# miguelmartin75/txt2vid

Measured on AMD Instinct MI355X. Metric: TGANv2 GAN train throughput (G+D steps x global batch), 16x64x64 videos/sec, higher is better.
Workload: dtype f32; 1 GPU; BASELINE configs[1]: unconditional TGANv2 16x64x64x1, per-GPU batch 32, fp32, RSGAN + GP 0.5, Adam 2e-4 (0.5,0.999), 1 D + 1 G step, subsample_input pyramid 8/16/32/64; global_batch=32, per_gpu_batch=32, parallelism=dp1

## Files before the change

include/t2v_hip.h:

```cpp
#ifndef T2V_HIP_H
#define T2V_HIP_H

#include <stddef.h>
#include <stdint.h>

#ifdef __cplusplus
extern "C" {
#endif

#define T2V_OK 0
#define T2V_EINVAL (-1)
#define T2V_ELAUNCH (-2)

#define T2V_MAX_TAPS 27

typedef struct {
    int32_t N, Cin, D, H, W, Cout;
    int32_t ntaps;
    int8_t dz[T2V_MAX_TAPS], dy[T2V_MAX_TAPS], dx[T2V_MAX_TAPS];
    int8_t pad_[3];
} t2v_conv_geom;

#define T2V_MAX_GROUPS 8
typedef struct {
// ... 53 lines not shown
typedef struct {
    const float* slab;
    const float* bias_slab;
    int32_t ntaps, S;
    int8_t map[T2V_MAX_TAPS];
    int8_t pad_[5];
    int64_t tap_stride;
    int64_t split_stride;
} t2v_wgrad_src;
typedef struct {
    float* dw;
    float* dbias;
    int64_t CoCi;
    int32_t T, Cout, nsrc;
    int32_t accum, accum_bias;
    int32_t kind;
    int32_t block_begin, nblocks;
    int32_t tap_major;
    int32_t pad_;
    t2v_wgrad_src src[T2V_WGRAD_MAX_SRC];
} t2v_wgrad_dest;
int t2v_conv_wgrad_grouped_partial(const t2v_conv_group* groups, int ngroups, int Cin, int Cout, int kD, int kH, int kW,
                                   float* slab, int want_bias, int flags, t2v_wgrad_src* out_src, void* stream);
int t2v_wgrad_dest_bytes(void);
int t2v_wgrad_reduce_multi(const void* table , int ndest, int total_blocks, void* stream);

int t2v_conv_fwd_plan(const t2v_conv_group* groups, int ngroups, int Cin, int Cout, int flags, int32_t* out);
int t2v_conv_wgrad_plan(const t2v_conv_group* groups, int ngroups, int Cin, int Cout, int kD, int kH, int kW, int32_t* out);
int64_t t2v_conv_wgrad_grouped_bias_slab_floats(const t2v_conv_group* groups, int ngroups, int Cin, int Cout, int kD,
                                                int kH, int kW);
int t2v_conv_wgrad_grouped_bias(const t2v_conv_group* groups, int ngroups, int Cin, int Cout, int kD, int kH, int kW,
                                float* dw, float* dbias, float* slab, int flags, void* stream);

int t2v_pack_weight_bf16(const float* w, void* wpb, int Cout, int Cin, int T, const int32_t* taps, int ntaps, int mode, void* stream);
int t2v_conv_fwd_grouped_bf16_ok(const t2v_conv_group* groups, int ngroups, int Cin, int Cout);
int t2v_conv_fwd_bf16_plan(const t2v_conv_group* groups, int ngroups, int Cin, int Cout, int flags, int32_t* out);
int t2v_conv_fwd_grouped_bf16(const t2v_conv_group* groups, int ngroups, int Cin, int Cout, const void* wpb, const float* bias,
                              float* ws, int flags, void* stream);

int64_t t2v_channel_sum_ws_floats(int N, int C, int64_t S);
int t2v_channel_sum(const float* x, float* out, float* ws, int N, int C, int64_t S, int accum, void* stream);
int64_t t2v_channel_sum_grouped_ws_floats(const t2v_conv_group* groups, int ngroups, int C);
int t2v_channel_sum_grouped(const t2v_conv_group* groups, int ngroups, int C, float* out, float* ws, int accum, void* stream);

int t2v_relu(const float* x, float* y, int64_t n, void* stream);
int t2v_relu_mask(const float* g, const float* x, float* gx, int64_t n, void* stream);
int t2v_add(const float* a, const float* b, float* y, int64_t n, void* stream);
int t2v_axpby(float alpha, const float* a, float beta, const float* b, float* y, int64_t n, void* stream);
int t2v_fill(float* y, float v, int64_t n, void* stream);
int t2v_tanh(const float* x, float* y, int64_t n, void* stream);
int t2v_tanh_bwd(const float* g, const float* y, float* gx, int64_t n, void* stream);

int t2v_avgpool3d(const float* x, const float* x2, float* y, int NC, int D, int H, int W, int Do, int Ho, int Wo,
                  const int32_t k[3], const int32_t s[3], const int32_t p[3], void* stream);
int t2v_avgpool3d_bwd(const float* gy, float* gx, int NC, int D, int H, int W, int Do, int Ho, int Wo,
                      const int32_t k[3], const int32_t s[3], const int32_t p[3], void* stream);
typedef struct t2v_pool_job {
    const float* x; const float* x2; float* y;
    const float* add;
    int32_t NC, D, H, W, Do, Ho, Wo;
    int32_t k[3], s[3], p[3];
} t2v_pool_job;
int t2v_avgpool3d_multi(const t2v_pool_job* jobs, int njobs, void* stream);
int t2v_avgpool3d_bwd_multi(const t2v_pool_job* jobs, int njobs, void* stream);

int t2v_rowsum(const float* x, float* y, int64_t rows, int64_t S, void* stream);
// ... 293 lines not shown
```

txt2vid_amd/_lib.py:

```python
import ctypes as C
import os

_HERE = os.path.dirname(os.path.abspath(__file__))
LIB_PATH = os.environ.get('T2V_LIB') or os.path.join(_HERE, 'csrc', 'libt2v_hip.so')

MAX_TAPS = 27


class ConvGeom(C.Structure):
    _fields_ = [('N', C.c_int32), ('Cin', C.c_int32), ('D', C.c_int32), ('H', C.c_int32), ('W', C.c_int32),
                ('Cout', C.c_int32), ('ntaps', C.c_int32),
                ('dz', C.c_int8 * MAX_TAPS), ('dy', C.c_int8 * MAX_TAPS), ('dx', C.c_int8 * MAX_TAPS),
                ('pad_', C.c_int8 * 3)]


class ConvGroup(C.Structure):
    _fields_ = [('x', C.c_void_p), ('y', C.c_void_p), ('mask', C.c_void_p), ('N', C.c_int32), ('D', C.c_int32), ('H', C.c_int32), ('W', C.c_int32),
                ('ntaps', C.c_int32), ('dstride', C.c_int32), ('ydstride', C.c_int32), ('yoff', C.c_int32), ('Dy', C.c_int32),
                ('dz', C.c_int8 * MAX_TAPS), ('dy', C.c_int8 * MAX_TAPS), ('dx', C.c_int8 * MAX_TAPS), ('widx', C.c_int8 * MAX_TAPS)]


class AdamJob(C.Structure):
    _fields_ = [('p', C.c_void_p), ('g', C.c_void_p), ('m', C.c_void_p), ('v', C.c_void_p), ('n', C.c_int64)]

# ... 78 lines not shown
_L = C.c_int64
_F = C.c_float
_I3 = C.POINTER(C.c_int32)
_G = C.POINTER(ConvGeom)

SIGNATURES = {
    't2v_pack_weight': [_P, _P, _I, _I, _I, _I3, _I, _I, _P],
    't2v_pack_job_bytes': [],
    't2v_pack_multi': [_P, _I, _I, _P],
    't2v_pack_job_groups': [_I, _I, _I],
    't2v_pack_weight_into': [_P, _P, _I, _I, _I, _I3, _I, _I, _I, _I, _I, _I, _P],
    't2v_conv_fwd': [_P, _P, _P, _P, _P, _G, _I, _P],
    't2v_conv_fwd_ws_floats': [_G],
    't2v_conv_wgrad_slab_floats': [_G, _I],
    't2v_conv_fwd_grouped_ws_floats': [_P, _I, _I, _I],
    't2v_conv_fwd_grouped': [_P, _I, _I, _I, _P, _P, _P, _I, _P],
    't2v_conv_wgrad_grouped_slab_floats': [_P, _I, _I, _I, _I, _I, _I],
    't2v_conv_fwd_plan': [_P, _I, _I, _I, _I, _I3],
    't2v_nonlocal_ok': [_I, _I],
    't2v_nonlocal_fwd': [_P, _P, _P, _P, _P, _I, _I, _I, _I, _I, _P],
    't2v_nonlocal_bwd': [_P, _P, _P, _P, _P, _P, _P, _P, _P, _P, _I, _I, _I, _I, _I, _P],
    't2v_conv_wgrad_grouped_partial': [_P, _I, _I, _I, _I, _I, _I, _P, _I, _I, _P, _P],
    't2v_wgrad_dest_bytes': [],
    't2v_wgrad_reduce_multi': [_P, _I, _I, _P],
    't2v_conv_wgrad_plan': [_P, _I, _I, _I, _I, _I, _I, _I3],
    't2v_pack_weight_bf16': [_P, _P, _I, _I, _I, _P, _I, _I, _P],
    't2v_conv_fwd_grouped_bf16_ok': [_P, _I, _I, _I],
    't2v_conv_fwd_bf16_plan': [_P, _I, _I, _I, _I, _I3],
    't2v_conv_fwd_grouped_bf16': [_P, _I, _I, _I, _P, _P, _P, _I, _P],
    't2v_conv_wgrad_grouped': [_P, _I, _I, _I, _I, _I, _I, _P, _P, _I, _P],
    't2v_conv_wgrad_grouped_bias_slab_floats': [_P, _I, _I, _I, _I, _I, _I],
    't2v_conv_wgrad_grouped_bias': [_P, _I, _I, _I, _I, _I, _I, _P, _P, _P, _I, _P],
    't2v_conv_wgrad': [_P, _P, _P, _P, _G, _I3, _I, _I, _P],
    't2v_channel_sum_ws_floats': [_I, _I, _L],
    't2v_channel_sum': [_P, _P, _P, _I, _I, _L, _I, _P],
    't2v_channel_sum_grouped_ws_floats': [_P, _I, _I],
    't2v_channel_sum_grouped': [_P, _I, _I, _P, _P, _I, _P],
    't2v_relu': [_P, _P, _L, _P],
    't2v_relu_mask': [_P, _P, _P, _L, _P],
    't2v_add': [_P, _P, _P, _L, _P],
    't2v_axpby': [_F, _P, _F, _P, _P, _L, _P],
    't2v_fill': [_P, _F, _L, _P],
    't2v_tanh': [_P, _P, _L, _P],
    't2v_tanh_bwd': [_P, _P, _P, _L, _P],
    't2v_avgpool3d': [_P, _P, _P, _I, _I, _I, _I, _I, _I, _I, _I3, _I3, _I3, _P],
    't2v_avgpool3d_bwd': [_P, _P, _I, _I, _I, _I, _I, _I, _I, _I3, _I3, _I3, _P],
    't2v_avgpool3d_multi': [_P, _I, _P],
    't2v_avgpool3d_bwd_multi': [_P, _I, _P],
    't2v_rowsum': [_P, _P, _L, _L, _P],
    't2v_rowbcast': [_P, _P, _L, _L, _P],
    't2v_upsample2x': [_P, _P, _L, _I, _I, _P],
    't2v_upsample2x_bwd': [_P, _P, _L, _I, _I, _P],
    't2v_upsample2x_add': [_P, _P, _P, _L, _I, _I, _P],
    't2v_rsgan_mean_multi': [_P, _I, _P, _P],
    't2v_rsgan_mean_multi_bwd': [_P, _I, _P, _P],
    't2v_bn_ws_floats': [_I, _I, _L],
    't2v_bn_plan': [_I, _I, _L, _I3],
    't2v_bn_stats': [_P, _P, _P, _P, _P, _I, _I, _L, _F, _F, _P],
    't2v_bn_apply': [_P, _P, _P, _P, _P, _I, _I, _L, _I, _P],
    't2v_bn_bwd': [_P, _P, _P, _P, _P, _P, _P, _P, _P, _I, _I, _L, _I, _P],
    't2v_bn_train_fwd': [_P, _P, _P, _P, _P, _P, _P, _P, _I, _I, _L, _F, _F, _I, _P, _P],
    't2v_bn_train_bwd': [_P, _P, _P, _P, _P, _P, _P, _P, _P, _I, _I, _L, _I, _P],
    't2v_bn_train_fwd_up': [_P, _P, _P, _P, _P, _P, _P, _P, _I, _I, _I, _I, _F, _F, _I, _P, _P],
    't2v_bn_train_bwd_up': [_P, _P, _P, _P, _P, _P, _P, _P, _P, _I, _I, _I, _I, _I, _P],
    't2v_bn_train_bwd_add': [_P, _P, _P, _P, _P, _P, _P, _P, _P, _P, _I, _I, _I, _I, _I, _I, _P],
    't2v_bn_eval': [_P, _P, _P, _P, _P, _P, _I, _I, _L, _F, _I, _P],
# ... 74 lines not shown
    't2v_pool_conv_plan': [_I, _P, _I, _I, _I, _I3],
    't2v_synth_clips': [_P, _I, _L, _I, _I, _I, _I3, _P, _P, _P, _P],
    't2v_clip_gather': [_P, _L, _P, _I, _I, _I, _I, _I, _P, _P, _P, _P],
    't2v_tseed_fwd_bn': [_P, _P, _P, _P, _P, _P, _P, _P, _P, _P, _P, _I, _I, _I, _I, _I, _F, _F, _I, _P],
    't2v_tseed_fwd_tanh': [_P, _P, _P, _P, _P, _I, _I, _I, _I, _P],
    't2v_tseed_bwd': [_P, _P, _P, _P, _P, _P, _P, _P, _P, _P, _I, _I, _I, _I, _I, _I, _P],
    't2v_ca_fwd': [_P, _P, _P, _P, _P, _I, _I, _I, _P],
    't2v_ca_bwd': [_P, _P, _F, _P, _P, _P, _I, _I, _I, _P],
    't2v_diffaug_fwd': [_P, _I, _P],
    't2v_diffaug_bwd': [_P, _I, _P],
    't2v_diffaug_gated_fwd': [_P, _P, _I, _P, _P],
    't2v_diffaug_gated_bwd': [_P, _P, _I, _P, _P],
    't2v_ada_update': [_P, _P, _I, _F, _F, _I, _P],
    't2v_lecam_fwd': [_P, _P, _I, _F, _I, _P, _P, _P],
    't2v_lecam_bwd': [_P, _I, _P, _P, _P],
    't2v_proj_rows': [_P, _I, _P, _I, _I, _P],
    't2v_proj_feat': [_P, _I, _P, _I, _I, _P],
    't2v_proj_cond': [_P, _I, _P, _I, _I, _P],
    't2v_proj_weight': [_P, _I, _P, _I, _I, _I, _P],
    't2v_mbstd_fwd': [_P, _I, _P, _I, _I, _I, _P],
    't2v_mbstd_feat': [_P, _I, _P, _I, _I, _I, _P],
    't2v_mbstd_second': [_P, _I, _P, _I, _I, _I, _P],
    't2v_mbstd_weight': [_P, _I, _P, _I, _I, _I, _I, _P],
    't2v_kid_sums': [_P, _P, _I, _I, _I, C.c_double, _P, _P, _P],
    't2v_kid_sums_ws_bytes': [_I, _I, _I],
    't2v_knn_radii': [_P, _I, _I, _I, _P, _P, _P],
    't2v_knn_radii_ws_bytes': [_I, _I, _I],
    't2v_prdc_counts': [_P, _P, _I, _I, _I, _P, _P, _P, _P, _P],
    't2v_prdc_counts_ws_bytes': [_I, _I, _I],
    't2v_prof_begin': [_I],
    't2v_prof_end': [C.POINTER(C.c_double), _I],
    't2v_version': [],
}
_RESTYPE = {'t2v_kid_sums_ws_bytes': C.c_size_t, 't2v_knn_radii_ws_bytes': C.c_size_t, 't2v_prdc_counts_ws_bytes': C.c_size_t, 't2v_multi_ws_floats': C.c_int64, 't2v_sn_ws_floats': C.c_int64, 't2v_pool_conv_fwd_ws_floats': C.c_int64, 't2v_pool_conv_wgrad_slab_floats': C.c_int64, 't2v_conv_wgrad_slab_floats': C.c_int64, 't2v_conv_wgrad_grouped_bias_slab_floats': C.c_int64, 't2v_conv_fwd_grouped_ws_floats': C.c_int64,
            't2v_conv_wgrad_grouped_slab_floats': C.c_int64, 't2v_conv_fwd_ws_floats': C.c_int64, 't2v_channel_sum_ws_floats': C.c_int64, 't2v_channel_sum_grouped_ws_floats': C.c_int64, 't2v_bn_ws_floats': C.c_int64, 't2v_cbn_ws_floats': C.c_int64, 't2v_version': C.c_char_p}

_lib = None


class T2VError(RuntimeError):
    pass


def lib():
    global _lib
    if _lib is None:
        if not os.path.exists(LIB_PATH):
            raise T2VError('libt2v_hip.so is missing (%s): run `python -c "import __graft_entry__ as g; g.build()"` '
                           'or `make -C txt2vid_amd/csrc`. There is no CPU/PyTorch fallback.' % LIB_PATH)
        import torch
        l = C.CDLL(LIB_PATH)
        for name, argtypes in SIGNATURES.items():
            fn = getattr(l, name)
            fn.argtypes = argtypes
            fn.restype = _RESTYPE.get(name, C.c_int)
        _lib = l
    return _lib


def check(status, what):
    if status != 0:
        raise T2VError('%s failed with status %d' % (what, status))
```

txt2vid_amd/csrc/conv.hip:

```cpp
#include <hip/hip_runtime.h>
#include <stdint.h>
#include "../../include/t2v_hip.h"

typedef float f32x16 __attribute__((ext_vector_type(16)));

#ifdef T2V_STAMPS
__device__ unsigned long long* g_stamps = nullptr;
__device__ unsigned int g_stamps_cap = 0;
extern "C" int t2v_stamps_set(void* buf, unsigned int cap_records) {
    if (hipMemcpyToSymbol(HIP_SYMBOL(g_stamps), &buf, sizeof(buf)) != hipSuccess) return -1;
    if (hipMemcpyToSymbol(HIP_SYMBOL(g_stamps_cap), &cap_records, sizeof(cap_records)) != hipSuccess) return -1;
    return 0;
}
__device__ __forceinline__ unsigned long long stamp_now() {
    unsigned long long t;
    __builtin_amdgcn_sched_barrier(0);
    asm volatile("s_memtime %0\n\ts_waitcnt lgkmcnt(0)" : "=s"(t) :: "memory");
    __builtin_amdgcn_sched_barrier(0);
    return t;
}
#define STAMP(v) const unsigned long long v = stamp_now()
#define STAMP_ACC(acc, a, b) acc += (b) - (a)
#else
#define STAMP(v)
// ... 3532 lines not shown
                acc = __builtin_amdgcn_mfma_f32_32x32x2f32(a4[i].w, b4[i].w, acc, 0, 0, 0);
            }
        }
        __syncthreads();
    }
    float* red = As;
    if (wk == 1) {
#pragma unroll
        for (int r = 0; r < 16; ++r) red[(wco * 16 + r) * 64 + lane] = acc[r];
    }
    __syncthreads();
    if (wk == 0) {
#pragma unroll
        for (int r = 0; r < 16; ++r) acc[r] += red[(wco * 16 + r) * 64 + lane];
        const int col = l31;
        if (col < ncols) {
            const int slot = col / Cin, ci = col - slot * Cin;
            float* ps = slab + ((size_t)split * live.n + slot) * Cout * Cin + ci;
#pragma unroll
            for (int r = 0; r < 16; ++r) {
                const int co = co0 + wco * 32 + (r & 3) + 8 * (r >> 2) + 4 * hi;
                if (co < Cout) ps[(size_t)co * Cin] = acc[r];
            }
        } else if (col == 31 && bias_slab != nullptr) {
#pragma unroll
            for (int r = 0; r < 16; ++r) {
                const int co = co0 + wco * 32 + (r & 3) + 8 * (r >> 2) + 4 * hi;
                if (co < Cout) bias_slab[(size_t)split * Cout + co] = acc[r];
            }
        }
    }
}

#define W3_AP (WG_BK + 1)
#define W3_BP (WG_BK + 3)
struct LiveRows { int8_t r[9]; int32_t n; };

#define W3_XP (WG_BK + 3)

template <bool BF16>
__global__ __launch_bounds__(256, BF16 ? 4 : 0) void conv_wgrad3_kernel(const WGroupTable tab, float* __restrict__ slab, const int Cin,
                                                          const int Cout, const int kD, const int kH, const int flags,
                                                          const int chunks_per_split, const LiveRows live,
                                                          float* __restrict__ bias_slab) {
    constexpr int LDS_A = BF16 ? 64 * B16_KP * 2 : 64 * W3_AP * 4;
    constexpr int LDS_B = BF16 ? 3 * 64 * B16_KP * 2 : 3 * 64 * W3_XP * 4;
    __shared__ __attribute__((aligned(16))) unsigned char lds_raw[LDS_A + LDS_B];
    float* const As = reinterpret_cast<float*>(lds_raw);
    float* const Bs = reinterpret_cast<float*>(lds_raw + LDS_A);
    __bf16* const Ah = reinterpret_cast<__bf16*>(lds_raw);
    __bf16* const Bh = reinterpret_cast<__bf16*>(lds_raw + LDS_A);
    const int tid = threadIdx.x, lane = tid & 63, wave = tid >> 6;
    const int l31 = lane & 31, hi = lane >> 5;
    const int wco = wave & 1, wci = wave >> 1;
    const int nco_t = (Cout + 63) / 64;
    const int co0 = (blockIdx.x % nco_t) * 64, ci0 = (blockIdx.x / nco_t) * 64;
    const int lin = xcd_remap((int)(blockIdx.y + blockIdx.z * gridDim.y), (int)(gridDim.y * gridDim.z));
    const int rslot = lin % (int)gridDim.y;
    const int split = lin / (int)gridDim.y;
    const int krow = live.r[rslot];
    const int dz = krow / kH - kD / 2, dy = krow % kH - kH / 2;
    const float relu_floor = (flags & T2V_CONV_RELU_IN) ? 0.f : -__builtin_inff();
    const int ml = tid & 31, rl = tid >> 5;
    const bool full = co0 + 64 <= Cout && ci0 + 64 <= Cin;

    f32x16 acc0, acc1, acc2;
// ... 566 lines not shown
        __syncthreads();
    }
    float* out = slab + (size_t)split * Cout * Cin;
#pragma unroll
    for (int i = 0; i < 2; ++i)
#pragma unroll
        for (int j = 0; j < 2; ++j) {
            const int ci = ci0 + wci * 64 + j * 32 + l31;
#pragma unroll
            for (int r = 0; r < 16; ++r) {
                const int co = co0 + wco * 64 + i * 32 + (r & 3) + 8 * (r >> 2) + 4 * hi;
                if (co < Cout && ci < Cin) out[(size_t)co * Cin + ci] = acc[i][j][r];
            }
        }
    if (do_bias) {
        float* red = As;
        *reinterpret_cast<float4*>(&red[r8 * WGM_AP + c4]) = bsum;
        __syncthreads();
        if (tid < 128 && co0 + tid < Cout) {
            float v = 0.f;
#pragma unroll
            for (int k = 0; k < 8; ++k) v += red[k * WGM_AP + tid];
            bias_slab[(size_t)split * Cout + co0 + tid] = v;
        }
    }
}

enum class WgradKernel {
    Taps = 0,
    Cols = 1,
    Rows3 = 2,
    Gemm = 3,
    Thin = 4,
    PoolRows3 = 11
};
struct WgradLaunch {
    WgradKernel kernel;
    bool bf16;
    bool strided;
    int S, cps;
    long nchunks;
    uint32_t live, liverows;
    int nlive, nrows;
    dim3 grid, block;
    bool reduce_small;
    int64_t slab_floats, bias_floats;
};

static long wgrad_ksplit(long base, long nch, long min_cps) {
    const long wg_target = tun().wgrad_target ? tun().wgrad_target : 1024;
    long S = base >= 1024 ? 1 : (wg_target + base - 1) / base;
    const long maxS = (nch + min_cps - 1) / min_cps;
    if (S > maxS) S = maxS;
    if (S < 1) S = 1;
    if (S > tun().wgrad_scap) S = tun().wgrad_scap;
    const long rounds = (base * S) / 1024, tail = (base * S) % 1024;
    if (tun().wgrad_quantise && rounds >= 1 && tail > 0 && tail * 5 <= 1024 && (rounds * 1024) / base >= 1) S = (rounds * 1024) / base;
    return S;
}
static void wgrad_set_splits(WgradLaunch& d, long S, int cps_multiple, int Cin, int Cout) {
    const long cps = ((d.nchunks + S - 1) / S + cps_multiple - 1) / cps_multiple * cps_multiple;
    d.cps = (int)cps;
    d.S = (int)((d.nchunks + cps - 1) / cps);
    d.grid.z = (unsigned)d.S;
    d.block = dim3(256);
    d.reduce_small = (long)Cout * Cin <= 16384 && d.S >= 16;
// ... 180 lines not shown
            else T2V_LAUNCH_PROF(conv_wgrad3_kernel<false>, d.grid, d.block, 0, s, tab, slab, Cin, Cout, kD, kH, flags, d.cps, lrows, bias_part);
            break;
        case WgradKernel::Thin:
            T2V_LAUNCH_PROF(conv_wgrad_thin_kernel, d.grid, d.block, 0, s, tab, slab, Cin, Cout, T, kH, kW, flags, d.cps, live, bias_part);
            break;
        case WgradKernel::Cols:
            T2V_LAUNCH_PROF(conv_wgrad_cols_kernel, d.grid, d.block, 0, s, tab, slab, Cin, Cout, T, kH, kW, flags, d.cps, live, bias_part);
            break;
        default:
            if (d.bf16) T2V_LAUNCH_PROF(conv_wgrad_bf16_kernel, d.grid, d.block, 0, s, tab, slab, Cin, Cout, T, kH, kW, flags, d.cps, live, bias_part);
            else T2V_LAUNCH_PROF(conv_wgrad_kernel, d.grid, d.block, 0, s, tab, slab, Cin, Cout, T, kH, kW, flags, d.cps, live, bias_part);
        }
    }
    int st = launch_status();
    if (st) return st;
    return wgrad_finish(d, T, map, slab, bias_part, dw, dbias, Cin, Cout, flags, s, out_src);
}
extern "C" int t2v_conv_wgrad_grouped(const t2v_conv_group* groups, int ngroups, int Cin, int Cout, int kD, int kH, int kW,
                                      float* dw, float* slab, int flags, void* stream) {
    return wgrad_impl(groups, ngroups, Cin, Cout, kD, kH, kW, dw, nullptr, false, slab, flags, stream, nullptr);
}
extern "C" int t2v_conv_wgrad_grouped_bias(const t2v_conv_group* groups, int ngroups, int Cin, int Cout, int kD, int kH, int kW,
                                           float* dw, float* dbias, float* slab, int flags, void* stream) {
    if (!dbias) return T2V_EINVAL;
    return wgrad_impl(groups, ngroups, Cin, Cout, kD, kH, kW, dw, dbias, true, slab, flags, stream, nullptr);
}

extern "C" int t2v_conv_wgrad_grouped_partial(const t2v_conv_group* groups, int ngroups, int Cin, int Cout, int kD, int kH,
                                              int kW, float* slab, int want_bias, int flags, t2v_wgrad_src* out_src,
                                              void* stream) {
    if (!out_src) return T2V_EINVAL;
    return wgrad_impl(groups, ngroups, Cin, Cout, kD, kH, kW, nullptr, nullptr, want_bias != 0, slab, flags, stream, out_src);
}
enum class PoolKernel { Fwd = 9, Dgrad = 10 };
struct PoolLaunch {
    PoolKernel kernel;
    bool db;
    bool vecb;
    int S;
    long tiles;
    dim3 grid, block;
    int64_t ws_floats;
};
static bool pool_member_ok(const t2v_conv_group& g, bool need_ptrs) {
    if (need_ptrs && (!g.x || !g.y)) return false;
    if (g.N < 1 || g.H < 2 || g.W < 2 || (g.H & 1) || (g.W & 1)) return false;
    if (g.dstride == 0) return g.D == 1;
    if (g.dstride != 1 && g.dstride != 2) return false;
    return g.D >= 2 && !(g.D & 1);
}
static inline long pool_rows(const t2v_conv_group& g) { return (long)g.N * (g.dstride ? g.D / 2 : 1) * (g.H / 2) * (g.W / 2); }
static inline long pool_padded(const t2v_conv_group& g) { return (long)(g.dstride ? g.D + 1 : 1) * (g.H + 1) * (g.W + 2); }
static inline long pool_grid(const t2v_conv_group& g) { return (long)(g.dstride ? g.D / 2 + 1 : 1) * (g.H / 2 + 1) * (g.W / 2 + 1); }
static inline long pool_grid_rows(const t2v_conv_group& g) { return (long)g.N * pool_grid(g); }

static bool decide_pool_fwd(const t2v_conv_group* groups, int ngroups, int Cin, int Cout, bool need_ptrs, GroupTable& tab, PoolLaunch& d) {
    if (!groups || ngroups < 1 || ngroups > T2V_MAX_GROUPS || Cin < 32 || (Cin % 32) || Cout < 4 || (Cout % 4)) return false;
    long ot = 0;
    int max_rows = 1;
    tab.n = ngroups;
    for (int i = 0; i < ngroups; ++i) {
        const t2v_conv_group& g = groups[i];
        if (!pool_member_ok(g, need_ptrs)) return false;
        if ((long)g.N * pool_padded(g) * Cin >= (1L << 29) || pool_rows(g) * Cout >= (1L << 31)) return false;
        if (g.ntaps != 9 && g.ntaps != 27) return false;
        if (g.dstride == 0 && g.ntaps != 9) return false;
// ... 549 lines not shown
```

txt2vid_amd/functional.py:

```python
import contextlib
import ctypes as C
import os
import weakref

import torch
from torch.autograd import Function
from torch.autograd.function import once_differentiable

from ._lib import lib, check, ConvGeom, ConvGroup, PackJob, WgradSrc, WgradDest, WGRAD_MAX_SRC, MAX_TAPS, MAX_GROUPS

FLAG_BIAS, FLAG_RELU_IN, FLAG_ACCUM, FLAG_MASK_OUT, FLAG_ACCUM_BIAS, FLAG_BF16 = 1, 2, 4, 8, 16, 32


from ._ops import _stream, _p, _c


def tap_major(w):
    nd = w.dim()
    fwd = tuple(range(2, nd)) + (0, 1)
    back = tuple(range(nd - 2, nd)) + tuple(range(nd - 2))
    return w.permute(*fwd).contiguous().permute(*back)


def is_tap_major(w):
    if w.is_contiguous():
        return False
    nd = w.dim()
    if nd >= 3 and w.permute(*(tuple(range(2, nd)) + (0, 1))).is_contiguous():
        return True
    raise ValueError('conv weights are dense [Cout,Cin,*k] or tap-major; got strides %s for shape %s' % (w.stride(), tuple(w.shape)))


def tap_rows(t):
    nd = t.dim()
    v = t.permute(*(tuple(range(2, nd)) + (0, 1)))
    return v.reshape(-1, t.shape[0] * t.shape[1])


_param_grads_enabled = True
WEIGHT_EPOCH = 0


@contextlib.contextmanager
def input_grads_only():
    global _param_grads_enabled
    old = _param_grads_enabled
    _param_grads_enabled = False
    try:
        yield
    finally:
        _param_grads_enabled = old


_NO_VEC_REDUCE = bool(os.environ.get('T2V_NO_VEC_REDUCE'))


class _PendingDest(object):
    __slots__ = ('wid', 'bid', 'dw', 'dbias', 'CoCi', 'T', 'Cout', 'accum', 'accum_bias', 'srcs', 'keep', 'tap_major')


class GradSink(object):

    def __init__(self, arenas):
        self.slots, self.count = {}, {}
        for arena in arenas:
            for off, p in zip(arena.offsets, arena.params):
                self.slots[id(p)] = (arena, off, p.numel())
        self.defer = os.environ.get('T2V_NO_DEFERRED_REDUCE') is None
        self.pending, self.pending_bias = {}, {}
        self.tables = {}
        self.slot_bytes, self.nslots = 65536, 48
        dev = arenas[0].flat.device if arenas else None
        self.tab_pin = self.tab_dev = None
        if dev is not None and dev.type == 'cuda' and self.defer:
            self.tab_pin = torch.empty(self.slot_bytes * self.nslots, dtype=torch.uint8).pin_memory()
            self.tab_dev = torch.empty(self.slot_bytes * self.nslots, dtype=torch.uint8, device=dev)
        else:
            self.defer = False
        self.ws, self.ws_off, self.ws_used = None, 0, 0
        self.frozen = 0

    def reset(self):
        self.flush()
        self.count.clear()
        grow = self.ws_used > (self.ws.numel() if self.ws is not None else 0)
        if grow and self.frozen:
            raise RuntimeError('the gradient sink would have to grow its slab workspace (%d -> %d floats) while a captured HIP graph '
# ... 1881 lines not shown
    else:
        wp = packed_weight(w5, ts, mode)
        check(lib().t2v_conv_fwd_grouped(arr, n, cin, cout, _p(wp), _p(bias), _p(ws), flags, _stream()), 't2v_conv_fwd_grouped')


def conv_group_raw(xs5, w5, bias=None, relu_in=False, mode=0, masks=None, outs=None, accum=False, even_frames=False):
    if len(xs5) > MAX_GROUPS:
        raise ValueError('at most %d tensors per grouped convolution' % MAX_GROUPS)
    if even_frames and (mode != 0 or masks is not None or accum or outs is not None):
        raise ValueError('even_frames is a plain forward option')
    xs5 = [_c(t) for t in xs5]
    w5 = _c(w5)
    Cout_w, Cin_w = w5.shape[0], w5.shape[1]
    cin, cout = (Cin_w, Cout_w) if mode == 0 else (Cout_w, Cin_w)
    ys = outs if outs is not None else [torch.empty((t.shape[0], cout, (t.shape[2] + 1) // 2 if even_frames else t.shape[2]) + tuple(t.shape[3:]),
                                                    device=t.device, dtype=torch.float32) for t in xs5]
    if masks is not None:
        masks = [_c(m) for m in masks]
        if any(m.shape != y.shape for m, y in zip(masks, ys)):
            raise ValueError('mask / output shape mismatch')
    arr, ts = _conv_table(xs5, ys, cin, cout, tuple(w5.shape[2:]), masks, 2 if even_frames else 0)
    ws = _fwd_workspace(arr, len(xs5), cin, cout, xs5[0].device)
    flags = ((FLAG_BIAS if bias is not None else 0) | (FLAG_RELU_IN if relu_in else 0) | (FLAG_MASK_OUT if masks is not None else 0) |
             (FLAG_ACCUM if accum else 0))
    _launch_group_fwd(arr, len(xs5), cin, cout, w5, ts, mode, bias, ws, flags)
    return ys


def _wgrad_table(xs5, gys5, wshape, want_bias, even_frames, sink=None):
    Cout, Cin = wshape[0], wshape[1]
    k = tuple(wshape[2:])
    geoms = [conv_geom(t.shape[0], Cin, t.shape[2], t.shape[3], t.shape[4], Cout, k[0], k[1], k[2]) for t in xs5]
    arr = _group_table(xs5, gys5, geoms, None, None, 2 if even_frames else 0)
    query = lib().t2v_conv_wgrad_grouped_bias_slab_floats if want_bias else lib().t2v_conv_wgrad_grouped_slab_floats
    n = int(query(arr, len(xs5), Cin, Cout, k[0], k[1], k[2]))
    if n <= 0:
        raise RuntimeError('bad grouped wgrad geometry')
    slab = sink.alloc_slab(n, xs5[0].device) if sink is not None else torch.empty((n,), device=xs5[0].device, dtype=torch.float32)
    return arr, slab


def conv_group_wgrad_raw(xs5, gys5, wshape, relu_in=False, out=None, accum=False, dbias=None, accum_bias=False, even_frames=False):
    xs5, gys5 = [_c(t) for t in xs5], [_c(t) for t in gys5]
    Cout, Cin = wshape[0], wshape[1]
    k = tuple(wshape[2:])
    arr, slab = _wgrad_table(xs5, gys5, wshape, dbias is not None, even_frames)
    dw = out if out is not None else torch.empty(tuple(wshape), device=xs5[0].device, dtype=torch.float32)
    flags = (FLAG_RELU_IN if relu_in else 0) | (FLAG_ACCUM if accum else 0) | (FLAG_BF16 if CONV_PRECISION == 'bf16' else 0)
    if dbias is not None:
        check(lib().t2v_conv_wgrad_grouped_bias(arr, len(xs5), Cin, Cout, k[0], k[1], k[2], _p(dw), _p(dbias), _p(slab),
                                                flags | (FLAG_ACCUM_BIAS if accum_bias else 0), _stream()),
              't2v_conv_wgrad_grouped_bias')
    else:
        check(lib().t2v_conv_wgrad_grouped(arr, len(xs5), Cin, Cout, k[0], k[1], k[2], _p(dw), _p(slab), flags, _stream()),
              't2v_conv_wgrad_grouped')
    return dw


def _wgrad_partial_launch(xs5, gys5, wshape, relu_in, want_bias, sink=None, even_frames=False):
    xs5, gys5 = [_c(t) for t in xs5], [_c(t) for t in gys5]
    Cout, Cin = wshape[0], wshape[1]
    k = tuple(wshape[2:])
    arr, slab = _wgrad_table(xs5, gys5, wshape, want_bias, even_frames, sink)
    src = WgradSrc()
    flags = (FLAG_RELU_IN if relu_in else 0) | (FLAG_BF16 if CONV_PRECISION == 'bf16' else 0)
    check(lib().t2v_conv_wgrad_grouped_partial(arr, len(xs5), Cin, Cout, k[0], k[1], k[2], _p(slab), 1 if want_bias else 0, flags,
                                               C.byref(src), _side.fork(xs5, gys5) if sink is not None else _stream()),
          't2v_conv_wgrad_grouped_partial')
    return src, slab


def _fused_gates_to_sink(sink, gates, x5, gy5, w4shape):
    Cc = w4shape[1]
    T = w4shape[2] * w4shape[3] * w4shape[4]
    src, slab = _wgrad_partial_launch([x5], [gy5], w4shape, False, False, sink)
    out = []
    for g, w in enumerate(gates):
        flat, acc = sink.take(w, deferred=True)
        sg = WgradSrc()
        C.memmove(C.byref(sg), C.byref(src), C.sizeof(WgradSrc))
        sg.slab = src.slab + 4 * g * Cc * Cc
        sink.add_partial(w, flat, acc, None, None, False, sg, slab, T, Cc, Cc * Cc, tap_major=True)
        out.append(None if acc else flat.as_strided(w.shape, w.stride()))
    return out


def zeros(shape, device, dtype=torch.float32):
    dev = torch.device(device)
    if dev.type != 'cuda' or dtype != torch.float32:
        return torch.zeros(shape, device=dev, dtype=dtype)
    out = torch.empty(shape, device=dev, dtype=dtype)
    if out.numel():
        check(lib().t2v_fill(_p(out), 0.0, out.numel(), _stream()), 't2v_fill')
    return out


def zeros_like(t):
    if not t.is_cuda or t.dtype != torch.float32:
        return torch.zeros_like(t, memory_format=torch.preserve_format)
    out = torch.empty_like(t, memory_format=torch.preserve_format)
    if out.numel():
# ... 415 lines not shown
```

Before: 3081 videos/s.

## Add specialized weight-gradient kernel for convolutions with few output channels

Adds a dedicated wgrad kernel for 3D convolutions with Cout ≤ 4, such as the RGB/mono output convs in the generator and the discriminator heads. Each wave keeps several input channels and a group of taps in registers, reduces across the DPP row and then shared memory, and splits voxels across blocks into a slab that the existing reduce pass finishes. The Python side routes eligible layers to the new path and keeps the old one when even_frames is set or inputs are large. This targets the poor utilization of the GEMM-style wgrad when the output dimension is tiny, at the cost of another code path and extra slab memory.

Result: no change. 3109 videos/s, median of 6 (+0.9%).

```diff
diff --git a/include/t2v_hip.h b/include/t2v_hip.h
--- a/include/t2v_hip.h
+++ b/include/t2v_hip.h
@@ -109,6 +109,15 @@
 int t2v_conv_wgrad_grouped_bias(const t2v_conv_group* groups, int ngroups, int Cin, int Cout, int kD, int kH, int kW,
                                 float* dw, float* dbias, float* slab, int flags, void* stream);
 
+int t2v_conv_wgrad_fewout_ok(const t2v_conv_group* groups, int ngroups, int Cin, int Cout, int kD, int kH, int kW);
+int t2v_conv_wgrad_fewout_plan(const t2v_conv_group* groups, int ngroups, int Cin, int Cout, int kD, int kH, int kW, int32_t* out);
+int64_t t2v_conv_wgrad_fewout_slab_floats(const t2v_conv_group* groups, int ngroups, int Cin, int Cout, int kD, int kH, int kW,
+                                          int want_bias);
+int t2v_conv_wgrad_fewout_partial(const t2v_conv_group* groups, int ngroups, int Cin, int Cout, int kD, int kH, int kW, float* slab,
+                                  int want_bias, int flags, t2v_wgrad_src* out_src, void* stream);
+int t2v_conv_wgrad_fewout(const t2v_conv_group* groups, int ngroups, int Cin, int Cout, int kD, int kH, int kW, float* dw,
+                          float* dbias, float* slab, int flags, void* stream);
+
 int t2v_pack_weight_bf16(const float* w, void* wpb, int Cout, int Cin, int T, const int32_t* taps, int ntaps, int mode, void* stream);
 int t2v_conv_fwd_grouped_bf16_ok(const t2v_conv_group* groups, int ngroups, int Cin, int Cout);
 int t2v_conv_fwd_bf16_plan(const t2v_conv_group* groups, int ngroups, int Cin, int Cout, int flags, int32_t* out);
diff --git a/txt2vid_amd/_lib.py b/txt2vid_amd/_lib.py
--- a/txt2vid_amd/_lib.py
+++ b/txt2vid_amd/_lib.py
@@ -134,6 +134,11 @@
     't2v_conv_wgrad_grouped_bias_slab_floats': [_P, _I, _I, _I, _I, _I, _I],
     't2v_conv_wgrad_grouped_bias': [_P, _I, _I, _I, _I, _I, _I, _P, _P, _P, _I, _P],
     't2v_conv_wgrad': [_P, _P, _P, _P, _G, _I3, _I, _I, _P],
+    't2v_conv_wgrad_fewout_ok': [_P, _I, _I, _I, _I, _I, _I],
+    't2v_conv_wgrad_fewout_plan': [_P, _I, _I, _I, _I, _I, _I, _I3],
+    't2v_conv_wgrad_fewout_slab_floats': [_P, _I, _I, _I, _I, _I, _I, _I],
+    't2v_conv_wgrad_fewout_partial': [_P, _I, _I, _I, _I, _I, _I, _P, _I, _I, _P, _P],
+    't2v_conv_wgrad_fewout': [_P, _I, _I, _I, _I, _I, _I, _P, _P, _P, _I, _P],
     't2v_channel_sum_ws_floats': [_I, _I, _L],
     't2v_channel_sum': [_P, _P, _P, _I, _I, _L, _I, _P],
     't2v_channel_sum_grouped_ws_floats': [_P, _I, _I],
@@ -274,7 +279,7 @@
     't2v_prof_end': [C.POINTER(C.c_double), _I],
     't2v_version': [],
 }
-_RESTYPE = {'t2v_kid_sums_ws_bytes': C.c_size_t, 't2v_knn_radii_ws_bytes': C.c_size_t, 't2v_prdc_counts_ws_bytes': C.c_size_t, 't2v_multi_ws_floats': C.c_int64, 't2v_sn_ws_floats': C.c_int64, 't2v_pool_conv_fwd_ws_floats': C.c_int64, 't2v_pool_conv_wgrad_slab_floats': C.c_int64, 't2v_conv_wgrad_slab_floats': C.c_int64, 't2v_conv_wgrad_grouped_bias_slab_floats': C.c_int64, 't2v_conv_fwd_grouped_ws_floats': C.c_int64,
+_RESTYPE = {'t2v_conv_wgrad_fewout_slab_floats': C.c_int64, 't2v_kid_sums_ws_bytes': C.c_size_t, 't2v_knn_radii_ws_bytes': C.c_size_t, 't2v_prdc_counts_ws_bytes': C.c_size_t, 't2v_multi_ws_floats': C.c_int64, 't2v_sn_ws_floats': C.c_int64, 't2v_pool_conv_fwd_ws_floats': C.c_int64, 't2v_pool_conv_wgrad_slab_floats': C.c_int64, 't2v_conv_wgrad_slab_floats': C.c_int64, 't2v_conv_wgrad_grouped_bias_slab_floats': C.c_int64, 't2v_conv_fwd_grouped_ws_floats': C.c_int64,
             't2v_conv_wgrad_grouped_slab_floats': C.c_int64, 't2v_conv_fwd_ws_floats': C.c_int64, 't2v_channel_sum_ws_floats': C.c_int64, 't2v_channel_sum_grouped_ws_floats': C.c_int64, 't2v_bn_ws_floats': C.c_int64, 't2v_cbn_ws_floats': C.c_int64, 't2v_version': C.c_char_p}
 
 _lib = None
diff --git a/txt2vid_amd/csrc/conv.hip b/txt2vid_amd/csrc/conv.hip
--- a/txt2vid_amd/csrc/conv.hip
+++ b/txt2vid_amd/csrc/conv.hip
@@ -3588,6 +3588,199 @@
     }
 }
 
+#define FO_TG 5
+#define FO_VOX 256
+template <int COUT> struct FewoutBlock { static constexpr int CB = COUT == 1 ? 8 : (COUT == 2 ? 4 : 2); };
+struct FewoutSlots { int32_t code[T2V_MAX_TAPS + FO_TG]; int32_t n; };
+
+__device__ __forceinline__ float fo_row_sum(float v) {
+    v += __builtin_bit_cast(float, __builtin_amdgcn_update_dpp(0, __builtin_bit_cast(int, v), 0xB1, 0xf, 0xf, true));
+    v += __builtin_bit_cast(float, __builtin_amdgcn_update_dpp(0, __builtin_bit_cast(int, v), 0x4E, 0xf, 0xf, true));
+    v += __builtin_bit_cast(float, __builtin_amdgcn_update_dpp(0, __builtin_bit_cast(int, v), 0x141, 0xf, 0xf, true));
+    v += __builtin_bit_cast(float, __builtin_amdgcn_update_dpp(0, __builtin_bit_cast(int, v), 0x140, 0xf, 0xf, true));
+    return v;
+}
+
+template <int COUT, bool VEC>
+__global__ __launch_bounds__(256, 2) void conv_wgrad_fewout_kernel(const WGroupTable tab, float* __restrict__ slab, const int Cin,
+                                                                   const int flags, const int rounds_per_split,
+                                                                   const FewoutSlots slots, float* __restrict__ bias_slab) {
+    constexpr int CB = FewoutBlock<COUT>::CB;
+    constexpr int NV = CB * FO_TG * COUT;
+    constexpr int NVT = NV + COUT;
+    __shared__ float red[4][4][NVT];
+    const int tid = threadIdx.x, lane = tid & 63, wave = tid >> 6;
+    const int ci0 = ((int)blockIdx.x * 4 + wave) * CB;
+    const int slot0 = (int)blockIdx.y * FO_TG;
+    const int split = blockIdx.z;
+    const float relu_floor = (flags & T2V_CONV_RELU_IN) ? 0.f : -__builtin_inff();
+
+    uint32_t need[FO_TG];
+    int scode[FO_TG];
+#pragma unroll
+    for (int j = 0; j < FO_TG; ++j) {
+        const int code = slots.code[slot0 + j];
+        scode[j] = code;
+        need[j] = code < 0 ? (1u << 9) : ((1u << (code & 3)) | (8u << ((code >> 2) & 3)) | (64u << ((code >> 4) & 3)));
+    }
+
+    float acc[CB][FO_TG][COUT];
+    float bsum[COUT];
+#pragma unroll
+    for (int c = 0; c < CB; ++c)
+#pragma unroll
+        for (int j = 0; j < FO_TG; ++j)
+#pragma unroll
+            for (int co = 0; co < COUT; ++co) acc[c][j][co] = 0.f;
+#pragma unroll
+    for (int co = 0; co < COUT; ++co) bsum[co] = 0.f;
+
+    const int nrounds = tab.chunk_start[tab.n];
+    const int q0 = split * rounds_per_split;
+    int q1 = q0 + rounds_per_split;
+    if (q1 > nrounds) q1 = nrounds;
+
+    int g_i = -1, g_begin = 0, g_end = 0;
+    int gD = 1, gH = 1, gW = 1, gHW = 1, gDHW = 1, gM = 0;
+    float r_dhw = 1.f, r_hw = 1.f, r_w = 1.f;
+    __amdgpu_buffer_rsrc_t g_x = __builtin_amdgcn_make_buffer_rsrc((void*)tab.g[0].x, 0, 0, 0x00020000);
+    __amdgpu_buffer_rsrc_t g_y = g_x;
+    auto enter_group = [&](int q) {
+        int gi = 0;
+#pragma unroll
+        for (int k = 1; k < T2V_MAX_GROUPS; ++k)
+            if (k < tab.n && q >= tab.chunk_start[k]) gi = k;
+        const t2v_conv_group& gd = tab.g[gi];
+        g_i = gi;
+        g_begin = tab.chunk_start[gi];
+        g_end = tab.chunk_start[gi + 1];
+        gD = gd.D; gH = gd.H; gW = gd.W; gHW = gH * gW; gDHW = gD * gHW; gM = gd.N * gDHW;
+        r_dhw = 1.0f / (float)gDHW; r_hw = 1.0f / (float)gHW; r_w = 1.0f / (float)gW;
+        g_x = __builtin_amdgcn_make_buffer_rsrc((void*)gd.x, 0, (int)((uint32_t)gM * (uint32_t)Cin * 4u), 0x00020000);
+        g_y = __builtin_amdgcn_make_buffer_rsrc((void*)gd.y, 0, (int)((uint32_t)gM * (uint32_t)COUT * 4u), 0x00020000);
+    };
+
+    for (int q = q0; q < q1; ++q) {
+        if (q >= g_end || g_i < 0) enter_group(q);
+        const int DHW = gDHW, HW = gHW, W = gW, H = gH, D = gD;
+        const uint32_t uDHW = (uint32_t)DHW;
+        const int mbase = (q - g_begin) * FO_VOX;
+        int soff[FO_TG];
+#pragma unroll
+        for (int j = 0; j < FO_TG; ++j)
+            soff[j] = ((scode[j] & 3) - 1) * HW + (((scode[j] >> 2) & 3) - 1) * W + (((scode[j] >> 4) & 3) - 1);
+
+        int mvox[4];
+        float xr[CB][4];
+        if constexpr (VEC) {
+            const int m = mbase + lane * 4;
+#pragma unroll
+            for (int e = 0; e < 4; ++e) mvox[e] = m + e;
+            const bool mv = m < gM;
+            const int mm = mv ? m : 0;
+            const int n = fast_div(mm, DHW, r_dhw), sp = mm - n * DHW;
+            const uint32_t xb = (uint32_t)(n * DHW) * (uint32_t)Cin + (uint32_t)sp;
+#pragma unroll
+            for (int c = 0; c < CB; ++c) {
+                const bool ok = mv & (ci0 + c < Cin);
+                const float4 v = __builtin_bit_cast(float4, __builtin_amdgcn_raw_buffer_load_b128(
+                    g_x, (ok ? xb + (uint32_t)(ci0 + c) * uDHW : 0u) * 4u, 0, 0));
+                xr[c][0] = ok ? fmaxf(v.x, relu_floor) : 0.f;
+                xr[c][1] = ok ? fmaxf(v.y, relu_floor) : 0.f;
+                xr[c][2] = ok ? fmaxf(v.z, relu_floor) : 0.f;
+                xr[c][3] = ok ? fmaxf(v.w, relu_floor) : 0.f;
+            }
+        } else {
+#pragma unroll
+            for (int e = 0; e < 4; ++e) {
+                const int m = mbase + e * 64 + lane;
+                mvox[e] = m;
+                const bool mv = m < gM;
+                const int mm = mv ? m : 0;
+                const int n = fast_div(mm, DHW, r_dhw), sp = mm - n * DHW;
+                const uint32_t xb = (uint32_t)(n * DHW) * (uint32_t)Cin + (uint32_t)sp;
+#pragma unroll
+                for (int c = 0; c < CB; ++c) {
+                    const bool ok = mv & (ci0 + c < Cin);
+                    const float v = __builtin_bit_cast(float, __builtin_amdgcn_raw_buffer_load_b32(
+                        g_x, (ok ? xb + (uint32_t)(ci0 + c) * uDHW : 0u) * 4u, 0, 0));
+                    xr[c][e] = ok ? fmaxf(v, relu_floor) : 0.f;
+                }
+            }
+        }
+
+#pragma unroll
+        for (int e = 0; e < 4; ++e) {
+            const int m = mvox[e];
+            const bool mv = m < gM;
+            const int mm = mv ? m : 0;
+            const int n = fast_div(mm, DHW, r_dhw), sp = mm - n * DHW;
+            const int d = fast_div(sp, HW, r_hw), r = sp - d * HW;
+            const int h = fast_div(r, W, r_w), w_ = r - h * W;
+            uint32_t vm = ((unsigned)(d - 1) < (unsigned)D ? 1u : 0u) | 2u | ((unsigned)(d + 1) < (unsigned)D ? 4u : 0u) |
+                          ((unsigned)(h - 1) < (unsigned)H ? 8u : 0u) | 16u | ((unsigned)(h + 1) < (unsigned)H ? 32u : 0u) |
+                          ((unsigned)(w_ - 1) < (unsigned)W ? 64u : 0u) | 128u | ((unsigned)(w_ + 1) < (unsigned)W ? 256u : 0u);
+            vm = mv ? vm : 0u;
+            const uint32_t yb = (uint32_t)(n * DHW) * (uint32_t)COUT + (uint32_t)sp;
+            float g[FO_TG][COUT];
+#pragma unroll
+            for (int j = 0; j < FO_TG; ++j) {
+                const bool ok = (vm & need[j]) == need[j];
+#pragma unroll
+                for (int co = 0; co < COUT; ++co) {
+                    const uint32_t off = ok ? (uint32_t)((int)(yb + (uint32_t)co * uDHW) + soff[j]) : 0u;
+                    const float v = __builtin_bit_cast(float, __builtin_amdgcn_raw_buffer_load_b32(g_y, off * 4u, 0, 0));
+                    g[j][co] = ok ? v : 0.f;
+                }
+            }
+#pragma unroll
+            for (int co = 0; co < COUT; ++co) {
+                const float v = __builtin_bit_cast(float, __builtin_amdgcn_raw_buffer_load_b32(
+                    g_y, (mv ? yb + (uint32_t)co * uDHW : 0u) * 4u, 0, 0));
+                bsum[co] += mv ? v : 0.f;
+            }
+#pragma unroll
+            for (int c = 0; c < CB; ++c)
+#pragma unroll
+                for (int j = 0; j < FO_TG; ++j)
+#pragma unroll
+                    for (int co = 0; co < COUT; ++co) acc[c][j][co] = fmaf(xr[c][e], g[j][co], acc[c][j][co]);
+            if constexpr (COUT >= 3) __builtin_amdgcn_sched_barrier(0);
+        }
+    }
+
+    const int row = lane >> 4;
+    const bool writer = (lane & 15) == 0;
+#pragma unroll
+    for (int c = 0; c < CB; ++c)
+#pragma unroll
+        for (int j = 0; j < FO_TG; ++j)
+#pragma unroll
+            for (int co = 0; co < COUT; ++co) {
+                const float v = fo_row_sum(acc[c][j][co]);
+                if (writer) red[wave][row][(c * FO_TG + j) * COUT + co] = v;
+            }
+#pragma unroll
+    for (int co = 0; co < COUT; ++co) {
+        const float v = fo_row_sum(bsum[co]);
+        if (writer) red[wave][row][NV + co] = v;
+    }
+    __syncthreads();
+    const int nlive = slots.n;
+    const bool do_bias = bias_slab != nullptr && blockIdx.x == 0 && blockIdx.y == 0;
+    for (int idx = tid; idx < 4 * NVT; idx += 256) {
+        const int wv = idx / NVT, k = idx - wv * NVT;
+        const float v = (red[wv][0][k] + red[wv][1][k]) + (red[wv][2][k] + red[wv][3][k]);
+        if (k < NV) {
+            const int co = k % COUT, j = (k / COUT) % FO_TG, c = k / (COUT * FO_TG);
+            const int ci = ((int)blockIdx.x * 4 + wv) * CB + c, slot = slot0 + j;
+            if (ci < Cin && slot < nlive) slab[(((size_t)split * nlive + slot) * COUT + co) * Cin + ci] = v;
+        } else if (do_bias && wv == 0) {
+            bias_slab[(size_t)split * COUT + (k - NV)] = v;
+        }
+    }
+}
+
 #define W3_AP (WG_BK + 1)
 #define W3_BP (WG_BK + 3)
 struct LiveRows { int8_t r[9]; int32_t n; };
@@ -4220,6 +4413,7 @@
     Rows3 = 2,
     Gemm = 3,
     Thin = 4,
+    Fewout = 5,
     PoolRows3 = 11
 };
 struct WgradLaunch {
@@ -4466,6 +4660,138 @@
     if (!out_src) return T2V_EINVAL;
     return wgrad_impl(groups, ngroups, Cin, Cout, kD, kH, kW, nullptr, nullptr, want_bias != 0, slab, flags, stream, out_src);
 }
+
+static bool decide_fewout(const t2v_conv_group* groups, int ngroups, int Cin, int Cout, int kD, int kH, int kW, bool need_ptrs,
+                          WGroupTable& tab, WgradLaunch& d, bool& vec) {
+    if (!groups || ngroups < 1 || ngroups > T2V_MAX_GROUPS || Cin < 1 || Cout < 1 || Cout > 4) return false;
+    if ((kD != 1 && kD != 3) || (kH != 1 && kH != 3) || (kW != 1 && kW != 3)) return false;
+    long nr = 0;
+    d.live = 0;
+    vec = true;
+    tab.n = ngroups;
+    for (int i = 0; i < ngroups; ++i) {
+        const t2v_conv_group& g = groups[i];
+        if (need_ptrs && (!g.x || !g.y)) return false;
+        if (g.N < 1 || g.D < 1 || g.H < 1 || g.W < 1) return false;
+        if (g.dstride < 0 || g.dstride > 1 || g.ydstride < 0 || g.ydstride > 1) return false;
+        if (voxels(g) * (long)(Cin > Cout ? Cin : Cout) >= (1L << 30)) return false;
+        if (voxels(g) >= (1L << 24)) return false;
+        vec = vec && (((long)g.D * g.H * g.W) & 3) == 0 && ((uintptr_t)g.x & 15) == 0;
+        tab.g[i] = g;
+        tab.chunk_start[i] = (int32_t)nr;
+        nr += (voxels(g) + FO_VOX - 1) / FO_VOX;
+        for (int a = 0; a < kD; ++a) for (int b = 0; b < kH; ++b) for (int c = 0; c < kW; ++c) {
+            const int dz = a - kD / 2, dy = b - kH / 2, dx = c - kW / 2;
+            if (!((g.D == 1 && dz) || (g.H == 1 && dy) || (g.W == 1 && dx))) d.live |= 1u << ((a * kH + b) * kW + c);
+        }
+    }
+    for (int i = ngroups; i <= T2V_MAX_GROUPS; ++i) tab.chunk_start[i] = (int32_t)nr;
+    const int cb4 = 4 * (Cout == 1 ? FewoutBlock<1>::CB : (Cout == 2 ? FewoutBlock<2>::CB : FewoutBlock<4>::CB));
+    d.kernel = WgradKernel::Fewout;
+    d.bf16 = false;
+    d.strided = false;
+    d.nchunks = nr;
+    d.nlive = __builtin_popcount(d.live);
+    d.liverows = 0;
+    d.nrows = 0;
+    const long base = (long)((Cin + cb4 - 1) / cb4) * ((d.nlive + FO_TG - 1) / FO_TG);
+    long S = (1024 + base - 1) / base;
+    if (S > 256) S = 256;
+    if (S > nr) S = nr;
+    if (S < 1) S = 1;
+    const long rps = (nr + S - 1) / S;
+    d.cps = (int)rps;
+    d.S = (int)((nr + rps - 1) / rps);
+    d.grid = dim3((unsigned)((Cin + cb4 - 1) / cb4), (unsigned)((d.nlive + FO_TG - 1) / FO_TG), (unsigned)d.S);
+    d.block = dim3(256);
+    d.reduce_small = (long)Cout * Cin <= 16384 && d.S >= 16;
+    d.slab_floats = (int64_t)d.S * d.nlive * Cout * Cin;
+    d.bias_floats = (int64_t)d.S * Cout;
+    return true;
+}
+extern "C" int t2v_conv_wgrad_fewout_ok(const t2v_conv_group* groups, int ngroups, int Cin, int Cout, int kD, int kH, int kW) {
+    WGroupTable tab;
+    WgradLaunch d;
+    bool vec;
+    return decide_fewout(groups, ngroups, Cin, Cout, kD, kH, kW, false, tab, d, vec) ? 1 : 0;
+}
+extern "C" int t2v_conv_wgrad_fewout_plan(const t2v_conv_group* groups, int ngroups, int Cin, int Cout, int kD, int kH, int kW,
+                                          int32_t* out) {
+    WGroupTable tab;
+    WgradLaunch d;
+    bool vec;
+    if (!out || !decide_fewout(groups, ngroups, Cin, Cout, kD, kH, kW, false, tab, d, vec)) return T2V_EINVAL;
+    wgrad_plan_out(d, out, 6);
+    return T2V_OK;
+}
+extern "C" int64_t t2v_conv_wgrad_fewout_slab_floats(const t2v_conv_group* groups, int ngroups, int Cin, int Cout, int kD, int kH,
+                                                     int kW, int want_bias) {
+    WGroupTable tab;
+    WgradLaunch d;
+    bool vec;
+    if (!decide_fewout(groups, ngroups, Cin, Cout, kD, kH, kW, false, tab, d, vec)) return T2V_EINVAL;
+    return d.slab_floats + (want_bias ? d.bias_floats : 0);
+}
+template <int COUT>
+static void fewout_launch(const WgradLaunch& d, bool vec, hipStream_t s, const WGroupTable& tab, float* slab, int Cin, int flags,
+                          const FewoutSlots& slots, float* bias_part) {
+    if (vec) T2V_LAUNCH_PROF((conv_wgrad_fewout_kernel<COUT, true>), d.grid, d.block, 0, s, tab, slab, Cin, flags, d.cps, slots, bias_part);
+    else T2V_LAUNCH_PROF((conv_wgrad_fewout_kernel<COUT, false>), d.grid, d.block, 0, s, tab, slab, Cin, flags, d.cps, slots, bias_part);
+}
+static int fewout_impl(const t2v_conv_group* groups, int ngroups, int Cin, int Cout, int kD, int kH, int kW, float* dw, float* dbias,
+                       bool want_bias, float* slab, int flags, int known_flags, void* stream, t2v_wgrad_src* out_src) {
+    WGroupTable tab;
+    WgradLaunch d;
+    bool vec;
+    if ((flags & ~known_flags) || (!dw && !out_src) || !slab) return T2V_EINVAL;
+    if (!decide_fewout(groups, ngroups, Cin, Cout, kD, kH, kW, true, tab, d, vec)) return T2V_EINVAL;
+    hipStream_t s = (hipStream_t)stream;
+    float* bias_part = want_bias ? slab + d.slab_floats : (float*)nullptr;
+    const int T = kD * kH * kW;
+    TapMap map;
+    FewoutSlots slots;
+    slots.n = 0;
+    for (int t = 0; t < T2V_MAX_TAPS; ++t) map.j[t] = -1;
+    for (int j = 0; j < T2V_MAX_TAPS + FO_TG; ++j) slots.code[j] = -1;
+    for (int t = 0; t < T; ++t)
+        if ((d.live >> t) & 1u) {
+            const int dz = t / (kH * kW) - kD / 2, dy = (t / kW) % kH - kH / 2, dx = t % kW - kW / 2;
+            map.j[t] = slots.n;
+            slots.code[slots.n++] = (1 - dz) | ((1 - dy) << 2) | ((1 - dx) << 4);
+        }
+    double flops = 0;
+    long M = 0;
+    for (int i = 0; i < ngroups; ++i) M += voxels(groups[i]);
+    flops = 2.0 * (double)M * Cout * Cin * d.nlive;
+    {
+        ProfScope prof(1, flops, s, M, Cin, Cout, d.nlive, ngroups, d.S);
+        int32_t plan_[8];
+        wgrad_plan_out(d, plan_, 8);
+        plan_[0] = -plan_[0];
+        ProfScope::set_plan(plan_, 8);
+        switch (Cout) {
+        case 1: fewout_launch<1>(d, vec, s, tab, slab, Cin, flags, slots, bias_part); break;
+        case 2: fewout_launch<2>(d, vec, s, tab, slab, Cin, flags, slots, bias_part); break;
+        case 3: fewout_launch<3>(d, vec, s, tab, slab, Cin, flags, slots, bias_part); break;
+        default: fewout_launch<4>(d, vec, s, tab, slab, Cin, flags, slots, bias_part);
+        }
+    }
+    int st = launch_status();
+    if (st) return st;
+    return wgrad_finish(d, T, map, slab, bias_part, dw, dbias, Cin, Cout, flags, s, out_src);
+}
+extern "C" int t2v_conv_wgrad_fewout(const t2v_conv_group* groups, int ngroups, int Cin, int Cout, int kD, int kH, int kW, float* dw,
+                                     float* dbias, float* slab, int flags, void* stream) {
+    if (!dw) return T2V_EINVAL;
+    return fewout_impl(groups, ngroups, Cin, Cout, kD, kH, kW, dw, dbias, dbias != nullptr, slab, flags,
+                       T2V_CONV_RELU_IN | T2V_CONV_ACCUM | T2V_CONV_ACCUM_BIAS | T2V_CONV_BF16, stream, nullptr);
+}
+extern "C" int t2v_conv_wgrad_fewout_partial(const t2v_conv_group* groups, int ngroups, int Cin, int Cout, int kD, int kH, int kW,
+                                             float* slab, int want_bias, int flags, t2v_wgrad_src* out_src, void* stream) {
+    if (!out_src) return T2V_EINVAL;
+    return fewout_impl(groups, ngroups, Cin, Cout, kD, kH, kW, nullptr, nullptr, want_bias != 0, slab, flags,
+                       T2V_CONV_RELU_IN | T2V_CONV_BF16, stream, out_src);
+}
 enum class PoolKernel { Fwd = 9, Dgrad = 10 };
 struct PoolLaunch {
     PoolKernel kernel;
diff --git a/txt2vid_amd/functional.py b/txt2vid_amd/functional.py
--- a/txt2vid_amd/functional.py
+++ b/txt2vid_amd/functional.py
@@ -53,6 +53,9 @@
 
 
 _NO_VEC_REDUCE = bool(os.environ.get('T2V_NO_VEC_REDUCE'))
+_NO_WGRAD_FEWOUT = os.environ.get('T2V_NO_WGRAD_FEWOUT') is not None
+FEWOUT_MIN_VOXELS = 512
+FEWOUT_MAX_INPUT_MULTI = 1 << 22
 
 
 class _PendingDest(object):
@@ -2000,22 +2003,34 @@
     k = tuple(wshape[2:])
     geoms = [conv_geom(t.shape[0], Cin, t.shape[2], t.shape[3], t.shape[4], Cout, k[0], k[1], k[2]) for t in xs5]
     arr = _group_table(xs5, gys5, geoms, None, None, 2 if even_frames else 0)
-    query = lib().t2v_conv_wgrad_grouped_bias_slab_floats if want_bias else lib().t2v_conv_wgrad_grouped_slab_floats
-    n = int(query(arr, len(xs5), Cin, Cout, k[0], k[1], k[2]))
+    fewout = False
+    if Cout <= 4 and not _NO_WGRAD_FEWOUT and not even_frames:
+        nx = sum(t.numel() for t in xs5)
+        fewout = (nx >= FEWOUT_MIN_VOXELS * Cin and (Cout == 1 or nx < FEWOUT_MAX_INPUT_MULTI)
+                  and lib().t2v_conv_wgrad_fewout_ok(arr, len(xs5), Cin, Cout, k[0], k[1], k[2]) == 1)
+    if fewout:
+        n = int(lib().t2v_conv_wgrad_fewout_slab_floats(arr, len(xs5), Cin, Cout, k[0], k[1], k[2], 1 if want_bias else 0))
+    else:
+        query = lib().t2v_conv_wgrad_grouped_bias_slab_floats if want_bias else lib().t2v_conv_wgrad_grouped_slab_floats
+        n = int(query(arr, len(xs5), Cin, Cout, k[0], k[1], k[2]))
     if n <= 0:
         raise RuntimeError('bad grouped wgrad geometry')
     slab = sink.alloc_slab(n, xs5[0].device) if sink is not None else torch.empty((n,), device=xs5[0].device, dtype=torch.float32)
-    return arr, slab
+    return arr, slab, fewout
 
 
 def conv_group_wgrad_raw(xs5, gys5, wshape, relu_in=False, out=None, accum=False, dbias=None, accum_bias=False, even_frames=False):
     xs5, gys5 = [_c(t) for t in xs5], [_c(t) for t in gys5]
     Cout, Cin = wshape[0], wshape[1]
     k = tuple(wshape[2:])
-    arr, slab = _wgrad_table(xs5, gys5, wshape, dbias is not None, even_frames)
+    arr, slab, fewout = _wgrad_table(xs5, gys5, wshape, dbias is not None, even_frames)
     dw = out if out is not None else torch.empty(tuple(wshape), device=xs5[0].device, dtype=torch.float32)
     flags = (FLAG_RELU_IN if relu_in else 0) | (FLAG_ACCUM if accum else 0) | (FLAG_BF16 if CONV_PRECISION == 'bf16' else 0)
-    if dbias is not None:
+    if fewout:
+        check(lib().t2v_conv_wgrad_fewout(arr, len(xs5), Cin, Cout, k[0], k[1], k[2], _p(dw), _p(dbias), _p(slab),
+                                          flags | (FLAG_ACCUM_BIAS if accum_bias and dbias is not None else 0), _stream()),
+              't2v_conv_wgrad_fewout')
+    elif dbias is not None:
         check(lib().t2v_conv_wgrad_grouped_bias(arr, len(xs5), Cin, Cout, k[0], k[1], k[2], _p(dw), _p(dbias), _p(slab),
                                                 flags | (FLAG_ACCUM_BIAS if accum_bias else 0), _stream()),
               't2v_conv_wgrad_grouped_bias')
@@ -2029,12 +2044,13 @@
     xs5, gys5 = [_c(t) for t in xs5], [_c(t) for t in gys5]
     Cout, Cin = wshape[0], wshape[1]
     k = tuple(wshape[2:])
-    arr, slab = _wgrad_table(xs5, gys5, wshape, want_bias, even_frames, sink)
+    arr, slab, fewout = _wgrad_table(xs5, gys5, wshape, want_bias, even_frames, sink)
     src = WgradSrc()
     flags = (FLAG_RELU_IN if relu_in else 0) | (FLAG_BF16 if CONV_PRECISION == 'bf16' else 0)
-    check(lib().t2v_conv_wgrad_grouped_partial(arr, len(xs5), Cin, Cout, k[0], k[1], k[2], _p(slab), 1 if want_bias else 0, flags,
-                                               C.byref(src), _side.fork(xs5, gys5) if sink is not None else _stream()),
-          't2v_conv_wgrad_grouped_partial')
+    partial = lib().t2v_conv_wgrad_fewout_partial if fewout else lib().t2v_conv_wgrad_grouped_partial
+    check(partial(arr, len(xs5), Cin, Cout, k[0], k[1], k[2], _p(slab), 1 if want_bias else 0, flags,
+                  C.byref(src), _side.fork(xs5, gys5) if sink is not None else _stream()),
+          't2v_conv_wgrad_fewout_partial' if fewout else 't2v_conv_wgrad_grouped_partial')
     return src, slab
 
 
```
